# weigert/SoilMachine

Hardware: NVIDIA H100
Metric: particle-steps/sec (higher is better)
Workload: dtype f64

## Files before the change

soilmachine_b200/csrc/sm_coop.cuh:

```cuda
#pragma once
#include "sm_core.cuh"

#if defined(__CUDA_ARCH__)
#define SM_POPC(x) __popc((unsigned int)(x))
#else
#define SM_POPC(x) __builtin_popcount((unsigned int)(x))
#endif

#define SM_CW_SLOTS 18
#define SM_CW_PLUS 186u

#define SM_BUDGET_SLOTS 6

template <class B, class = void> struct CellBudgetOf { static constexpr bool value = false; };
template <class B> struct CellBudgetOf<B, decltype(void(B::kCellBudget))> { static constexpr bool value = B::kCellBudget; };

struct
#if defined(__CUDACC__)
    __align__(32)
#else
    alignas(32)
#endif
        CoopScratch {
  Sec32 win[SM_CW_SLOTS];
  double hs[2][8];
  double d;
  uint32_t u;
  unsigned char ord[2][8];
  uint32_t pad_[3];
  double acc[SM_BUDGET_SLOTS];
  double pad2_[2];
};

struct WindField {
  const float* v4;
  int nx, ny, nz;
  int dimx, dimy, scale;
};
SM_HD void wind_field_pspeed(const WindField& f, float px, float py, double height, float* ps) {
  if (!f.v4) { ps[0] = -2.0f; ps[1] = 0.0f; ps[2] = 1.0f; return; }
  const float sx = (float)f.dimx / (float)f.nx, sy = (float)f.scale / 32.0f, sz = (float)f.dimy / (float)f.nz;
  int lx = (int)(px / sx), lz = (int)(py / sz);
  int ly = (int)((float)(height * 80.0 / (double)f.scale) * (float)f.scale / sy);
  lx = lx < 0 ? 0 : (lx > f.nx - 1 ? f.nx - 1 : lx);
  ly = ly < 0 ? 0 : (ly > f.ny - 1 ? f.ny - 1 : ly);
  lz = lz < 0 ? 0 : (lz > f.nz - 1 ? f.nz - 1 : lz);
  const float* v = f.v4 + (((size_t)lx * f.ny + ly) * f.nz + lz) * 4;
  for (int k = 0; k < 3; k++) {
    float c = v[k] / 0.05f;
    c = c < -2.0f ? -2.0f : (c > 2.0f ? 2.0f : c);
    ps[k] = c;
  }
}

template <class B> struct CoopWin {
  B& b;
  CoopScratch* s;
  int ax, ay, bx, by;
  uint32_t valid, dirtym;
  bool has_b;
  float f_freq, f_track;
  static constexpr bool kBudget = B::kBudget;
  static constexpr bool kCellBudget = CellBudgetOf<B>::value;
  SM_HD CoopWin(B& b_, CoopScratch* s_) : b(b_), s(s_), ax(0), ay(0), bx(0), by(0), valid(0), dirtym(0), has_b(false),
                                          f_freq(0.f), f_track(0.f) {}
  SM_HD int dimx() const { return b.dimx(); }
  SM_HD int dimy() const { return b.dimy(); }
  SM_HD int scale() const { return b.scale(); }
  SM_HD const SoilDev& soil(uint32_t t) const { return *b.soilp(t); }

  SM_HD int slot_of(int x, int y) const {
    int dx = x - ax + 1, dy = y - ay + 1;
    if ((unsigned)dx < 3u && (unsigned)dy < 3u) return dx * 3 + dy;
    if (has_b) {
      dx = x - bx + 1; dy = y - by + 1;
      if ((unsigned)dx < 3u && (unsigned)dy < 3u) return 9 + dx * 3 + dy;
    }
    return -1;
  }
  template <class W> SM_HD void fetch_a(W& w, uint32_t want) {
    const int nx_ = b.dimx(), ny_ = b.dimy();
    const uint32_t have = valid;
    const uint32_t got = w.ballot(9, [&](int k) {
      const int x = ax + k / 3 - 1, y = ay + k % 3 - 1;
      const bool need = ((want >> k) & 1u) && !((have >> k) & 1u) && x >= 0 && y >= 0 && x < nx_ && y < ny_;
      if (need) s->win[k] = *b.cell_ptr(x, y);
      return need;
    });
    valid |= got;
  }
  template <class W> SM_HD void begin(W& w, int ix, int iy, int kind, uint32_t mask = 0x1FFu) {
    ax = ix; ay = iy; has_b = false; valid = 0; dirtym = 0;
    const int ind = iy * b.dimx() + ix;
    if (kind == 0) { f_freq = b.wfreq(ind); f_track = b.wtrack(ind); }
    else f_freq = b.windfreq(ind);
    fetch_a(w, mask);
  }
  template <class W> SM_HD void target(W& w, int nx, int ny) {
    bx = nx; by = ny; has_b = true;
    const int nx_ = b.dimx(), ny_ = b.dimy();
    const uint32_t have = valid;
    const uint32_t got = w.ballot(18, [&](int l) {
      if (l < 9) {
        const int x = nx + l / 3 - 1, y = ny + l % 3 - 1;
        bool need = x >= 0 && y >= 0 && x < nx_ && y < ny_;
        const int dx = x - ax + 1, dy = y - ay + 1;
        if ((unsigned)dx < 3u && (unsigned)dy < 3u) need = false;
        if (need) s->win[9 + l] = *b.cell_ptr(x, y);
        return need;
      }
      const int k = l - 9;
      const int x = ax + k / 3 - 1, y = ay + k % 3 - 1;
      const int dx = x - nx + 1, dy = y - ny + 1;
      const bool need = !((have >> k) & 1u) && (unsigned)dx < 3u && (unsigned)dy < 3u && x >= 0 && y >= 0 && x < nx_ && y < ny_;
      if (need) s->win[k] = *b.cell_ptr(x, y);
      return need;
    });
    valid |= ((got & 0x1FFu) << 9) | (got >> 9);
  }
  SM_HD Sec32* rec(int x, int y) {
    const int sl = slot_of(x, y);
    return sl >= 0 ? &s->win[sl] : b.cell_ptr(x, y);
  }
  SM_HD double height(int x, int y) { return rec_height(*rec(x, y)); }
  SM_HD void dirty(int x, int y) {
    const int sl = slot_of(x, y);
    if (sl >= 0) dirtym |= 1u << sl;
  }
  SM_HD void dirty_rec(const Sec32* r) {
    const long off = (long)(r - s->win);
    if (off >= 0 && off < SM_CW_SLOTS) dirtym |= 1u << (int)off;
  }
  template <class W> SM_HD void touched(W& w, Sec32* r, int x, int y) {
    dirty_rec(r);
    if (B::kHydroHooks && w.lead()) b.air_mark(r, x, y);
  }
  SM_HD void detach() { ax = ay = bx = by = -(1 << 28); has_b = false; valid = 0; dirtym = 0; }
  SM_HD void dirty_rec(Sec32* r, int x, int y) { dirty_rec(r); if (B::kHydroHooks) b.air_mark(r, x, y); }
  SM_HD void wet_mark(int x, int y) { if (B::kHydroHooks) b.wet_mark(x, y); }
  SM_HD double volume_factor() const { return b.volume_factor(); }
  SM_HD void cell_budget(int term, int x, int y, double d) {
    if constexpr (kCellBudget) b.cell_budget(term, x, y, d);
  }
  template <class W> SM_HD void flush(W& w) {
    const uint32_t m = dirtym;
    w.each(SM_CW_SLOTS, [&](int l) {
      if ((m >> l) & 1u) {
        const int ox = l < 9 ? ax : bx, oy = l < 9 ? ay : by, k = l < 9 ? l : l - 9;
        *b.cell_ptr(ox + k / 3 - 1, oy + k % 3 - 1) = s->win[l];
      }
    });
    dirtym = 0;
  }
  SM_HD void focus(int x, int y) { b.focus(x, y); }
  SM_HD Sec32 pool_load(uint32_t i) { return b.pool_load(i); }
  SM_HD void pool_store(uint32_t i, const Sec32& r) { b.pool_store(i, r); }
  SM_HD uint32_t pool_alloc() { return b.pool_alloc(); }
  SM_HD void pool_free(uint32_t i) { b.pool_free(i); }
};

template <class A>
SM_HD bool cascade_eval(A& a, const Sec32* pc, const Sec32* pn, int SCALE, float& transfer, uint32_t& cascades,
                        bool& centre_top) {
  const double dd = (rec_height(*pc) - rec_height(*pn)) * (float)SCALE;
  const Sec32* const tr = (dd > 0) ? pc : pn;
  const SoilDev& sp = a.soil(rec_surface(*tr));
  if (fabs(dd) < 80.0 * (double)sp.maxdiff * (1.0 - 9.5367431640625e-07)) return false;
  const float diff = (float)(dd / 80.0f);
  if (diff == 0) return false;
  const float excess = fabsf(diff) - sp.maxdiff;
  if (excess <= 0) return false;
  transfer = sp.settling * excess / 2.0f;
  const double tsize = (tr->type == SM_EMPTY) ? 0.0 : tr->size;
  if (transfer > tsize) transfer = (float)tsize;
  cascades = sp.cascades;
  centre_top = dd > 0;
  return true;
}

template <int DEPTH, class W, class A> struct CascadeCoop {
  static SM_HD void run(W& w, A& a, int cx, int cy, int transferloop) {
    const int dimx = a.dimx(), dimy = a.dimy();
    const int SCALE = a.scale();
    double* const hs = a.s->hs[DEPTH];
    unsigned char* const ord = a.s->ord[DEPTH];
    const unsigned int inb = ((cx > 0 ? 0x07u : 0u) | 0x18u | (cx < dimx - 1 ? 0xE0u : 0u)) &
                             ((cy > 0 ? 0x29u : 0u) | 0x42u | (cy < dimy - 1 ? 0x94u : 0u));
    const int num = SM_POPC(inb);
    Sec32* const pc = a.rec(cx, cy);
    const unsigned int active = w.ballot(8, [&](int k) {
      if (!((inb >> k) & 1u)) { hs[k] = -1.0e300; return false; }
      const int kk = k + (k >= 4 ? 1 : 0);
      const Sec32* pn = a.rec(cx + kk / 3 - 1, cy + kk % 3 - 1);
      hs[k] = rec_height(*pn);
      float t; uint32_t cs; bool ct;
      return cascade_eval(a, pc, pn, SCALE, t, cs, ct);
    });
    if (active == 0) return;
    w.each(8, [&](int k) {
      const double hk = hs[k];
      int r = 0;
#pragma unroll
      for (int j = 0; j < 8; j++) {
        const double hj = hs[j];
        r += (j > k) ? (hj > hk ? 1 : 0) : ((j < k) ? (hk > hj ? 0 : 1) : 0);
      }
      ord[r] = (unsigned char)k;
    });
    int f = -1;
#pragma unroll
    for (int r = 7; r >= 0; r--) if (r < num && ((active >> ord[r]) & 1u)) f = r;
    for (;;) {
      const int k = (int)ord[f];
      const int kk = k + (k >= 4 ? 1 : 0);
      const int nx = cx + kk / 3 - 1, ny = cy + kk % 3 - 1;
      Sec32* const pn = a.rec(nx, ny);
      w.one([&]() {
        float transfer = 0.f; uint32_t casc = 0; bool ctop = false;
        cascade_eval(a, pc, pn, SCALE, transfer, casc, ctop);
        Sec32* const tr = ctop ? pc : pn;
        Sec32* const br = ctop ? pn : pc;
        a.b.note_transfer();
        double ht0 = 0.0, hb0 = 0.0;
        if (A::kBudget) { ht0 = rec_height(*tr); hb0 = rec_height(*br); }
        a.focus(ctop ? cx : nx, ctop ? cy : ny);
        const bool re = col_remove(a, *tr, (double)transfer) != 0;
        a.focus(ctop ? nx : cx, ctop ? ny : cy);
        col_add(a, *br, (double)transfer, casc);
        if (A::kBudget) {
          const double dt = rec_height(*tr) - ht0, db = rec_height(*br) - hb0;
          a.s->acc[2] += dt + db;
          a.cell_budget(2, ctop ? cx : nx, ctop ? cy : ny, dt);
          a.cell_budget(2, ctop ? nx : cx, ctop ? ny : cy, db);
        }
        a.s->u = re ? 1u : 0u;
      });
      a.touched(w, pc, cx, cy);
      a.touched(w, pn, nx, ny);
      if constexpr (DEPTH > 0) {
        const bool recascade = a.s->u != 0;
        if (recascade && transferloop > 0) {
          --transferloop;
          CascadeCoop<DEPTH - 1, W, A>::run(w, a, nx, ny, transferloop);
        }
      }
      const int start = f + 1;
      const unsigned int act = w.ballot(num, [&](int r) {
        if (r < start) return false;
        const int k2 = (int)ord[r];
        const int kk2 = k2 + (k2 >= 4 ? 1 : 0);
        const Sec32* pn2 = a.rec(cx + kk2 / 3 - 1, cy + kk2 % 3 - 1);
        float t; uint32_t cs; bool ct;
        return cascade_eval(a, pc, pn2, SCALE, t, cs, ct);
      });
      if (act == 0) return;
      f = SM_FFS(act) - 1;
    }
  }
};

struct WaterMidCoop {
  float freq, solubility, equrate;
  double evaprate;
  int ix, iy;
};
template <class W, class A> SM_HD int water_move_coop(W& w, A& a, WaterP& p, WaterMidCoop& m, uint32_t amask = 0x1FFu) {
  const int dimx = a.dimx(), dimy = a.dimy();
  if (A::kBudget && w.lead()) { for (int k = 0; k < SM_BUDGET_SLOTS; k++) a.s->acc[k] = 0.0; }
  const int ix = (int)roundf(p.px), iy = (int)roundf(p.py);
  a.begin(w, ix, iy, 0, amask);
  const sm_f3 n = map_normal(a, ix, iy);
  Sec32* const ir = a.rec(ix, iy);
  SoilDev param = a.soil(rec_surface(*ir));
  double evaprate = 0.01;
  const int ind = iy * dimx + ix;
  if (w.lead()) a.b.set_wtrack(ind, (float)(a.f_track + p.volume));
  const float freq = a.f_freq;
  param.friction = param.friction * (1.0f - freq);
  evaprate = evaprate * (1.0f - 0.2f * freq);
  m.freq = freq; m.solubility = param.solubility; m.equrate = param.equrate; m.evaprate = evaprate;
  m.ix = ix; m.iy = iy;
  {
    const float vx = n.x * param.friction, vz = n.z * param.friction;
    if (sqrtf(vx * vx + vz * vz) < 1E-5) return SM_EXIT_STALL;
  }
  {
    const float f = param.friction;
    const float mx = n.x * (1.0f - f) + p.sx * f;
    const float my = n.z * (1.0f - f) + p.sy * f;
    const float inv = 1.0f / sqrtf(mx * mx + my * my);
    p.sx = SM_SQRT2F * (mx * inv);
    p.sy = SM_SQRT2F * (my * inv);
  }
  p.px += p.sx;
  p.py += p.sy;
  if (!(p.px >= 0.0f && p.py >= 0.0f) ||
      !(p.px < (float)dimx - 1.0f && p.py < (float)dimy - 1.0f)) {
    if (A::kBudget && w.lead()) a.s->acc[3] += p.sediment * p.volume;
    p.volume = 0.0;
    return SM_EXIT_OOB;
  }
  return SM_ALIVE;
}
template <class W, class A> SM_HD int water_interact_coop(W& w, A& a, WaterP& p, const WaterMidCoop& m) {
  const int SCALE = a.scale();
  const int ix = m.ix, iy = m.iy;
  const float freq = m.freq;
  const double evaprate = m.evaprate;
  Sec32* const ir = a.rec(ix, iy);
  const int nx = (int)roundf(p.px), ny = (int)roundf(p.py);
  a.target(w, nx, ny);
  double c_eq = m.solubility * (rec_height(*ir) - map_height_bilinear(a, p.px, p.py)) *
                (double)SCALE / 80.0;
  if (c_eq < 0.0) c_eq = 0.0;
  if (c_eq > 1.0) c_eq = 1.0;
  if ((double)(a.soil(p.contains).erosionrate) < freq)
    p.contains = a.soil(p.contains).erodes;
  const double cdiff = c_eq - p.sediment;
  if (cdiff > 0) {
    p.sediment += m.equrate * cdiff;
    p.contains = a.soil(rec_surface(*ir)).transports;
    const double amount = m.equrate * cdiff * p.volume;
    w.one([&]() {
      const double h0 = A::kBudget ? rec_height(*ir) : 0.0;
      a.focus(ix, iy);
      double diff = col_remove(a, *ir, amount);
      SM_UNROLL1
      while (fabs(diff) > 1E-8) diff = col_remove(a, *ir, diff);
      if (A::kBudget) { const double d = h0 - rec_height(*ir); a.s->acc[0] += d; a.cell_budget(0, ix, iy, d); }
    });
    a.dirty_rec(ir);
  } else if (cdiff < 0) {
    const float eq = a.soil(p.contains).equrate;
    p.sediment += eq * cdiff;
    const double amount = -eq * cdiff * p.volume;
    const uint32_t what = p.contains;
    w.one([&]() {
      const double h0 = A::kBudget ? rec_height(*ir) : 0.0;
      a.focus(ix, iy);
      col_add(a, *ir, amount, what);
      if (A::kBudget) { const double d = rec_height(*ir) - h0; a.s->acc[1] += d; a.cell_budget(1, ix, iy, d); }
    });
    a.dirty_rec(ir);
  }
  CascadeCoop<0, W, A>::run(w, a, nx, ny, 0);
// ... 2 lines not shown
  if (p.sediment > 1.0) p.sediment = 1.0;
  p.volume *= (1.0 - evaprate);
  const bool lives = p.volume > 0.01;
  if (A::kBudget && w.lead()) {
    if (over > 0.0) a.s->acc[4] += over * p.volume;
    if (!lives) a.s->acc[3] += p.sediment * p.volume;
  }
  return lives ? SM_ALIVE : SM_EXIT_EVAP;
}
template <class W, class A> SM_HD int water_step_coop(W& w, A& a, WaterP& p, uint32_t amask = 0x1FFu) {
  WaterMidCoop m;
  const int r = water_move_coop(w, a, p, m, amask);
  if (r != SM_ALIVE) return r;
  return water_interact_coop(w, a, p, m);
}

struct WindMidCoop {
  float suspension;
  uint32_t transports;
  int ix, iy;
};
template <class W, class A> SM_HD int wind_move_coop(W& w, A& a, WindP& p, WindMidCoop& m, uint32_t amask = 0x1FFu) {
  const int dimx = a.dimx(), dimy = a.dimy();
  const int SCALE = a.scale();
  if (A::kBudget && w.lead()) { for (int k = 0; k < SM_BUDGET_SLOTS; k++) a.s->acc[k] = 0.0; }
  if (a.soil(p.contains).suspension == 0.0) return SM_EXIT_OOB;
  const int ix = (int)roundf(p.px), iy = (int)roundf(p.py);
  a.begin(w, ix, iy, 1, amask);
  const sm_f3 n = map_normal(a, ix, iy);
  Sec32* const ir = a.rec(ix, iy);
  const SoilDev& param = a.soil(rec_surface(*ir));
  m.suspension = param.suspension; m.transports = param.transports; m.ix = ix; m.iy = iy;
  if (w.lead()) a.b.set_windfreq(iy * dimx + ix, (float)(0.5 * a.f_freq + 0.5f));
  const double sheight = rec_height(*ir) * (float)SCALE / 80.0f;
  if (p.height < sheight) p.height = sheight;
  if (p.height > sheight) {
    p.sy = (float)(p.sy - 0.25);
  } else {
    const sm_f3 s{p.sx, p.sy, p.sz};
    const sm_f3 v = f3_cross(f3_cross(s, n), n);
    const double wt = 0.8;
    p.sx = (float)((double)s.x * (1.0 - wt) + (double)v.x * wt);
    p.sy = (float)((double)s.y * (1.0 - wt) + (double)v.y * wt);
    p.sz = (float)((double)s.z * (1.0 - wt) + (double)v.z * wt);
  }
  {
    float ps[3];
    a.b.pspeed(p.px, p.py, p.height, ps);
    const double wt = 0.2;
    p.sx = (float)((double)p.sx * (1.0 - wt) + (double)(ps[0]) * wt);
    p.sy = (float)((double)p.sy * (1.0 - wt) + (double)(ps[1]) * wt);
    p.sz = (float)((double)p.sz * (1.0 - wt) + (double)(ps[2]) * wt);
  }
  p.px += p.sx;
  p.py += p.sz;
  p.height += p.sy;
  if (!(p.px >= 0.0f && p.py >= 0.0f) ||
      !((int)p.px < dimx - 1 && (int)p.py < dimy - 1) ||
      sqrtf(p.sx * p.sx + p.sy * p.sy + p.sz * p.sz) < 0.01) {
    if (A::kBudget && w.lead()) a.s->acc[3] += p.sediment;
    return SM_EXIT_OOB;
  }
  return SM_ALIVE;
}
template <class W, class A> SM_HD int wind_interact_coop(W& w, A& a, WindP& p, const WindMidCoop& m) {
  const int SCALE = a.scale();
  const int ix = m.ix, iy = m.iy;
// ... 64 lines not shown
```

soilmachine_b200/csrc/sm_engine.cu:

```cuda
#include <cuda_runtime.h>
#include <stddef.h>
#include <stdio.h>
#include <stdlib.h>
#include <string.h>
#include <string>
#include <vector>
#include <algorithm>
#include "../../include/soilmachine_b200.h"
#include "../../include/soilmachine/soilfile.hpp"
#include "sm_device.cuh"
#include "sm_noise.cuh"
#include "sm_hydro.cuh"
#include "sm_lbm.cuh"
#include "sm_snap.cuh"
#include "sm_layer.cuh"
#include "sm_relax.cuh"
#include <cub/device/device_scan.cuh>
#include <type_traits>

#define KIND_WATER 0
#define KIND_WIND 1

template <int KIND> struct Reach {
  static constexpr int D = (KIND == KIND_WATER) ? 6 : 10;
// ... 1163 lines not shown
  HydroAccess a(c, s_soils, s_rec, s_tag, am, true);
  HydroCount hc{};
  const unsigned long long cells = am.ncells;
  for (unsigned long long cell = active_next(am, 0); cell < cells; cell = active_next(am, cell + 1))
    hydro_seep_visit(a, (int)(cell / (unsigned long long)c.dimy), (int)(cell % (unsigned long long)c.dimy), hc);
  a.flush();
  hydro_count_out(out, hc);
}

template <bool CELLS> struct HydroCellsRef {
  __device__ __forceinline__ explicit HydroCellsRef(double*) {}
};
template <> struct HydroCellsRef<true> {
  double* hcells;
  __device__ __forceinline__ explicit HydroCellsRef(double* m) : hcells(m) {}
};
struct FreqPeers {
  float* wfreq[SM_MAX_RANKS];
  float* wtrack[SM_MAX_RANKS];
};
template <bool MULTI> struct FreqPeersRef {
  __device__ __forceinline__ explicit FreqPeersRef(const FreqPeers*) {}
};
template <> struct FreqPeersRef<true> {
  const FreqPeers* fp;
  __device__ __forceinline__ explicit FreqPeersRef(const FreqPeers* f) : fp(f) {}
};
template <bool MULTI, bool BUDGET, bool CELLS = false>
struct HydroBack : DevBack<MULTI, BUDGET>, HydroCellsRef<CELLS>, FreqPeersRef<MULTI> {
  static_assert(!CELLS || BUDGET, "the per-cell maps are measured by the budget instantiations");
  static_assert(!(CELLS && MULTI), "the hydrology's per-cell maps are not kept on a sharded map");
  static constexpr bool kHydroHooks = true;
  static constexpr bool kCellBudget = CELLS;
  ActiveMap act;
  bool marking;
  __device__ __forceinline__ HydroBack(const DevCtx& ctx, const SoilDev* ss, const ActiveMap& am, bool mk,
                                       double* cells = nullptr, const FreqPeers* fp = nullptr)
      : DevBack<MULTI, BUDGET>(ctx, ss, 0u), HydroCellsRef<CELLS>(cells), FreqPeersRef<MULTI>(fp), act(am), marking(mk) {}
  __device__ __forceinline__ float wfreq(int i) const {
    if constexpr (MULTI) return this->fp->wfreq[owner_of_x<true>(this->c, i % this->c.dimx)][i];
    else return this->c.wfreq[i];
  }
  __device__ __forceinline__ float wtrack(int i) const {
    if constexpr (MULTI) return this->fp->wtrack[owner_of_x<true>(this->c, i % this->c.dimx)][i];
    else return this->c.wtrack[i];
  }
  __device__ __forceinline__ void set_wtrack(int i, float v) {
    if constexpr (MULTI) this->fp->wtrack[owner_of_x<true>(this->c, i % this->c.dimx)][i] = v;
    else this->c.wtrack[i] = v;
  }
  __device__ __forceinline__ void cell_budget(int term, int x, int y, double d) {
    if constexpr (CELLS) {
      double* const m = this->hcells + ((size_t)x * this->c.dimy + y) * SM_HYDRO_CELL_TERMS + term;
      __builtin_assume(__isGlobal(m));
      atomicAdd(m, d);
    }
  }
  __device__ __forceinline__ void air_mark(Sec32* r, int x, int y) {
    if (marking && r->type == SM_AIR) active_mark_block(act, x, y, this->c.dimx, this->c.dimy);
  }
  __device__ __forceinline__ void wet_mark(int x, int y) {
    if (marking) active_set(act, (unsigned long long)x * this->c.dimy + y);
  }
};
struct HydroTotals {
  HydroCount hc;
// ... 835 lines not shown
  bool use_coop = SM_DEFAULT_COOP || ctx->d.bud != nullptr || ctx->d.wind_v4 != nullptr;
  {
    const char* e = getenv("SM_KERNEL");
    if (e && strcmp(e, "thread") == 0) use_coop = false;
    if (e && strcmp(e, "warp") == 0) use_coop = true;
  }
  if (ctx->d_cells && !use_coop) ctx->cells_state = 2;
  else if (ctx->d_cells && ctx->cells_state == 0) ctx->cells_state = 1;
  if (use_coop) {
    const int sw_warps = kind == KIND_WIND ? SwShape<KIND_WIND>::WARPS : SwShape<KIND_WATER>::WARPS;
    const int cthreads = sw_warps * 32;
    int occ = 0;
    const bool budget = ctx->d.bud != nullptr;
    bool exact = false;
    {
      const char* e = getenv("SM_EXACT");
      exact = (((e ? atoi(e) : SM_DEFAULT_EXACT) >> kind) & 1) != 0;
    }
    void* const fns[16] = {(void*)k_sweep<KIND_WATER, false, false, false, false>, (void*)k_sweep<KIND_WIND, false, false, false, false>,
                           (void*)k_sweep<KIND_WATER, true, false, false, false>,  (void*)k_sweep<KIND_WIND, true, false, false, false>,
                           (void*)k_sweep<KIND_WATER, false, true, false, false>,  (void*)k_sweep<KIND_WIND, false, true, false, false>,
                           (void*)k_sweep<KIND_WATER, true, true, false, false>,   (void*)k_sweep<KIND_WIND, true, true, false, false>,
                           (void*)k_sweep<KIND_WATER, false, false, true, false>,  (void*)k_sweep<KIND_WIND, false, false, true, false>,
                           (void*)k_sweep<KIND_WATER, true, false, true, false>,   (void*)k_sweep<KIND_WIND, true, false, true, false>,
                           (void*)k_sweep<KIND_WATER, false, true, true, false>,   (void*)k_sweep<KIND_WIND, false, true, true, false>,
                           (void*)k_sweep<KIND_WATER, true, true, true, false>,    (void*)k_sweep<KIND_WIND, true, true, true, false>};
    void* const fns_cells[8] = {(void*)k_sweep<KIND_WATER, false, true, false, true>, (void*)k_sweep<KIND_WIND, false, true, false, true>,
                                (void*)k_sweep<KIND_WATER, true, true, false, true>,  (void*)k_sweep<KIND_WIND, true, true, false, true>,
                                (void*)k_sweep<KIND_WATER, false, true, true, true>,  (void*)k_sweep<KIND_WIND, false, true, true, true>,
                                (void*)k_sweep<KIND_WATER, true, true, true, true>,   (void*)k_sweep<KIND_WIND, true, true, true, true>};
    void* fn = ctx->d_cells ? fns_cells[(exact ? 4 : 0) + (multi ? 2 : 0) + (kind == KIND_WATER ? 0 : 1)]
                            : fns[(exact ? 8 : 0) + (budget ? 4 : 0) + (multi ? 2 : 0) + (kind == KIND_WATER ? 0 : 1)];
    const size_t csmem = (size_t)2 * (((size_t)std::max(n, 1) + 31) / 32) * sizeof(unsigned int);
    if (csmem > 40 * 1024) CK(cudaFuncSetAttribute((const void*)fn, cudaFuncAttributeMaxDynamicSharedMemorySize, (int)csmem));
    CK(cudaOccupancyMaxActiveBlocksPerMultiprocessor(&occ, (const void*)fn, cthreads, csmem));
    if (occ < 1) return fail(ctx, SM_ERR_CUDA, "sweep kernel does not fit an SM");
    const long long maxblocks = std::max<long long>(1, (long long)ctx->num_sms * occ / ctx->share);
    const long long want = ((long long)std::max(n, 1) + sw_warps - 1) / sw_warps;
    const int cblocks = (int)std::max<long long>(1, std::min(maxblocks, want));
    DevCtx dd = ctx->d;
    int ms = max_sweeps;
    if (ms <= 0) ms = -1;
    if (max_sweeps == SM_SWEEPS_NONE) ms = 0;
    CellMaps cm = ctx->cells_of;
    void* cargs[] = {&dd, &n, (void*)&d_spawn, &ms, &cm};
    CK(cudaMemsetAsync(ctx->d.ctl, 0, 4 * sizeof(unsigned int), ctx->stream));
    CK(cudaMemsetAsync(&ctx->d.ctl->ticket[0], 0, 3 * sizeof(unsigned int), ctx->stream));
    for (int i = 0; i < 3; i++)
      CK(cudaMemsetAsync(ctx->d.lmask[i], 0, ((size_t)ctx->max_particles / 32 + 2) * sizeof(unsigned int), ctx->stream));
    CK(cudaEventRecord(ctx->ev0, ctx->stream));
    CK(cudaLaunchCooperativeKernel(fn, dim3(cblocks), dim3(cthreads), cargs, csmem, ctx->stream));
    CK(cudaEventRecord(ctx->ev1, ctx->stream));
    ctx->launches++;
    ctx->timing_pending = true;
    return SM_OK;
  }
  DevCtx d = ctx->d;
  if (max_sweeps <= 0) max_sweeps = -1;
  if (max_sweeps == SM_SWEEPS_NONE) max_sweeps = 0;
  void* args[] = {&d, &n, (void*)&d_spawn, &max_sweeps, &lshift};
  CK(cudaMemsetAsync(ctx->d.ctl, 0, 4 * sizeof(unsigned int), ctx->stream));
  CK(cudaEventRecord(ctx->ev0, ctx->stream));
  if (multi && kind == KIND_WATER)
    CK(cudaLaunchCooperativeKernel((void*)k_run<KIND_WATER, true>, dim3(blocks), dim3(threads), args, smem, ctx->stream));
  else if (multi)
    CK(cudaLaunchCooperativeKernel((void*)k_run<KIND_WIND, true>, dim3(blocks), dim3(threads), args, smem, ctx->stream));
  else if (use_exact && kind == KIND_WATER)
// ... 1200 lines not shown
```

soilmachine_b200/csrc/sm_sweep.cuh:

```cuda
#pragma once
#include "sm_coop.cuh"

template <int KIND> struct SwShape {
  static constexpr int WARPS = (KIND == KIND_WIND) ? 10 : 8;
  static constexpr int MINBLOCKS = (KIND == KIND_WIND) ? 2 : 3;
};
#define SM_SW_NEAR 31
#define SM_SW_NEARX 128

struct WarpDev {
  int lane;
  template <class F> __device__ __forceinline__ void each(int n, F f) {
    __syncwarp();
    if (lane < n) f(lane);
    __syncwarp();
  }
  template <class F> __device__ __forceinline__ unsigned int ballot(int n, F f) {
    __syncwarp();
    bool v = false;
    if (lane < n) v = f(lane);
    const unsigned int m = __ballot_sync(0xffffffffu, v);
    __syncwarp();
    return m;
  }
  template <class F> __device__ __forceinline__ void one(F f) {
    __syncwarp();
    if (lane == 0) f();
    __syncwarp();
  }
  __device__ __forceinline__ bool lead() const { return lane == 0; }
};

struct CellMaps {
  double* p[SM_MAX_RANKS];
};

template <bool CELLS> struct CellMapsRef {
  __device__ __forceinline__ explicit CellMapsRef(const CellMaps*) {}
};
template <> struct CellMapsRef<true> {
  const CellMaps* cm;
  __device__ __forceinline__ explicit CellMapsRef(const CellMaps* m) : cm(m) {}
};

template <bool MULTI, bool BUDGET = false, bool CELLS = false> struct DevBack : CellMapsRef<CELLS> {
  static constexpr bool kBudget = BUDGET;
  static constexpr bool kHydroHooks = false;
  static constexpr bool kCellBudget = CELLS;
  __device__ __forceinline__ void air_mark(Sec32*, int, int) {}
  __device__ __forceinline__ void wet_mark(int, int) {}
  __device__ __forceinline__ double volume_factor() const { return c.volume_factor; }
  const DevCtx& c;
  const SoilDev* s_soils;
  unsigned int phase;
  int cur_q;
  __device__ __forceinline__ DevBack(const DevCtx& ctx, const SoilDev* ss, unsigned int tag, const CellMaps* m = nullptr)
      : CellMapsRef<CELLS>(m), c(ctx), s_soils(ss), phase(tag % 3u), cur_q(0) {}
  __device__ __forceinline__ void cell_budget(int term, int x, int y, double d) {
    const int q = owner_of_x<MULTI>(c, x);
    double* const m = this->cm->p[q];
    atomicAdd(m + ((size_t)(x - q * c.strip_w) * c.dimy + y) * 3 + term, d);
  }
  __device__ __forceinline__ int dimx() const { return c.dimx; }
  __device__ __forceinline__ int dimy() const { return c.dimy; }
// ... 23 lines not shown
    atomicAdd(&c.ctl->drops, 1ull);
    return SM_NIL;
  }
  __device__ void pool_free(uint32_t i) {
    RunCtl* const ctl = MULTI ? c.peer[cur_q].ctl : c.ctl;
    uint32_t* const ring = MULTI ? c.peer[cur_q].ringbuf[phase] : c.ringbuf[phase];
    const unsigned long long cap = MULTI ? c.peer[cur_q].pool_cap : c.pool_cap;
    PoolRing* R = &ctl->ring[phase];
    const unsigned long long t = MULTI ? atomicAdd_system(&R->tail, 1ull) : atomicAdd(&R->tail, 1ull);
    ring[t % cap] = i;
  }
  __device__ __forceinline__ float wfreq(int i) const { return c.wfreq[i]; }
  __device__ __forceinline__ float wtrack(int i) const { return c.wtrack[i]; }
  __device__ __forceinline__ float windfreq(int i) const { return c.windfreq[i]; }
  __device__ __forceinline__ void set_wtrack(int i, float v) { c.wtrack[i] = v; }
  __device__ __forceinline__ void set_windfreq(int i, float v) { c.windfreq[i] = v; }
  __device__ __forceinline__ void note_transfer() {}
  __device__ __forceinline__ void pspeed(float px, float py, double height, float* ps) const {
    const WindField f{c.wind_v4, c.wind_nx, c.wind_ny, c.wind_nz, c.dimx, c.dimy, c.scale};
    wind_field_pspeed(f, px, py, height, ps);
  }
};

struct __align__(32) WarpSmem {
  CoopScratch cs;
  uint32_t blk[SM_SW_NEARX];
  uint32_t pred[12];
  uint32_t cnt;
  uint32_t m0[SM_SW_NEARX / 32];
  uint32_t n1[SM_SW_NEARX / 32];
  uint32_t remote;
  uint32_t succ;
  uint32_t blkxy[SM_SW_NEARX];
};

#ifndef SM_PREFETCH
#define SM_PREFETCH 1
#endif
__device__ __forceinline__ float next_dy(const WaterP& p) { return p.sy; }
__device__ __forceinline__ float next_dy(const WindP& p) { return p.sz; }
template <class W, class A> __device__ __forceinline__ int do_step_coop(W& w, A& a, WaterP& p) { return water_step_coop(w, a, p); }
template <class W, class A> __device__ __forceinline__ int do_step_coop(W& w, A& a, WindP& p) { return wind_step_coop(w, a, p); }

template <int KIND, bool MULTI, bool EXACT = false>
__device__ __forceinline__ uint32_t coop_scan(const DevCtx& c, WarpSmem& ws, int lane, unsigned int tag, int pid, int ix,
                                              int iy, int R) {
  const unsigned int par = tag & 1u;
  const int G = Reach<KIND>::G;
  const int nbx = (c.dimx + G - 1) / G, nby = (c.dimy + G - 1) / G;
  if (lane == 0) { ws.cnt = 0; ws.succ = 0; if (EXACT) ws.remote = 0; }
  if (EXACT && lane < SM_SW_NEARX / 32) ws.m0[lane] = 0;
  __syncwarp();
  if (lane < 9) {
    const int cx = ix / G + lane / 3 - 1, cy = iy / G + lane % 3 - 1;
    uint32_t best = SM_NIL;
    if (cx >= 0 && cx < nbx && cy >= 0 && cy < nby) {
      const int bq = MULTI ? owner_of_x<MULTI>(c, cx * G) : 0;
      const unsigned long long* hp = MULTI ? c.peer[bq].head[par] : c.head[par];
      const unsigned long long h = *((volatile const unsigned long long*)&hp[cx * nby + cy]);
      if ((unsigned int)(h >> 32) == tag) {
        const uint2* nodes = MULTI ? c.peer[bq].node[par] : c.node[par];
        const uint32_t qtag = MULTI ? ((uint32_t)bq << 28) : 0u;
        uint32_t j = (uint32_t)h;
        while (j != SM_NIL) {
          const uint2 nd = nodes[j];
          if (j > (uint32_t)pid) ws.succ = 1u;
// ... 241 lines not shown
  for (int i = lo; i < hi; i++) { s_pref[i] = run; run += (unsigned int)__popc(s_word[i]); }
  __syncthreads();
  return total;
}

template <int KIND, bool MULTI, bool BUDGET, bool EXACT, bool CELLS>
__global__ void __launch_bounds__(SwShape<KIND>::WARPS * 32, SwShape<KIND>::MINBLOCKS) k_sweep(DevCtx c, int n, const float* __restrict__ spawn,
                                                                            int max_sweeps, const __grid_constant__ CellMaps cm) {
  typedef typename PType<KIND>::T P;
  constexpr int NWARPS = SwShape<KIND>::WARPS;
  __shared__ SoilDev s_soils[SM_MAX_SOILS];
  __shared__ unsigned int s_alive, s_total, s_wsum[NWARPS];
  __shared__ WarpSmem s_w[NWARPS];
  extern __shared__ unsigned int s_live[];
  const int W = (n + 31) >> 5;
  unsigned int* const s_word = s_live;
  unsigned int* const s_pref = s_live + W;
  for (int i = threadIdx.x; i < c.nsoils; i += blockDim.x) s_soils[i] = c.soils[i];
  if (threadIdx.x == 0) s_alive = 0;
  __syncthreads();

  RunCtl* ctl = c.ctl;
  unsigned int epoch = 0;
  const unsigned int tag0 = ctl->tag_base;
  const unsigned int gbase = MULTI ? ctl->epoch_base : 0u;
  const int gtid = blockIdx.x * blockDim.x + threadIdx.x;
  const int lane = threadIdx.x & 31;
  const int wib = threadIdx.x >> 5;
  const int slot = blockIdx.x * NWARPS + wib;
  const int nslots = gridDim.x * NWARPS;
  WarpSmem& ws = s_w[wib];
  WarpDev w{lane};

  unsigned long long n_steps = 0, n_oob = 0, n_evap = 0, n_stall = 0;
  bool any_doa = false;

  unsigned int total_alive = 0;
  {
    unsigned int my_alive = 0;
    unsigned long long doa = 0;
    const int nthreads = gridDim.x * blockDim.x;
    for (int pid = gtid; pid < n; pid += nthreads) {
      bool alive;
      if (spawn != nullptr) {
        const float x = spawn[2 * pid], y = spawn[2 * pid + 1];
        const int sx = (int)roundf(x), sy = (int)roundf(y);
        if (MULTI && owner_of_x<MULTI>(c, sx) != c.rank) {
          c.alive[pid] = 0;
          if (BUDGET) for (int k = 0; k < SM_BUDGET_SLOTS; k++) c.bud[(size_t)pid * SM_BUDGET_SLOTS + k] = 0.0;
          continue;
        }
        const uint32_t contains = s_soils[rec_surface(*cell_ptr<MULTI>(c, sx, sy))].transports;
        if (KIND == KIND_WATER) {
          WaterP q{x, y, 0.0f, 0.0f, 1.0, 0.0, contains};
          store_particle(c, pid, q);
          alive = true;
        } else {
          WindP q{x, y, -2.0f, 0.0f, 1.0f, 0.0, 0.0, contains};
          store_particle(c, pid, q);
          alive = !(s_soils[contains].suspension == 0.0);
          if (!alive) { doa++; any_doa = true; }
        }
        c.alive[pid] = alive ? 1 : 0;
        c.done[pid] = alive ? (tag0 - 1u) : 0xFFFFFFFFu;
        if (EXACT) c.fin[pid] = alive ? (tag0 - 1u) : 0xFFFFFFFFu;
        if (BUDGET) for (int k = 0; k < SM_BUDGET_SLOTS; k++) c.bud[(size_t)pid * SM_BUDGET_SLOTS + k] = 0.0;
      } else {
// ... 17 lines not shown
    if (MULTI) total_alive = grid_barrier_x(c, epoch, gbase, 0u, true, &s_total);
    else grid_barrier(&ctl->barrier, epoch);
  }
  const bool xnb = MULTI && c.strip_w >= 3 * Reach<KIND>::G;
  bool xglobal = true;
  int last_active = -1;

  int s = 0;
  for (;; s++) {
    const unsigned int tag = tag0 + (unsigned int)s;
    if (max_sweeps >= 0 && s >= max_sweeps) {
      if (!MULTI) total_alive = live_total<NWARPS>(c.lmask[tag % 3u], W, s_word, s_pref, s_wsum);
      break;
    }
    const unsigned int live = live_total<NWARPS>(c.lmask[tag % 3u], W, s_word, s_pref, s_wsum);
    if (!MULTI) total_alive = live;
    if ((!MULTI || xglobal) && total_alive == 0) break;
    {
      unsigned int* const z = c.lmask[(tag + 2u) % 3u];
      for (int i = gtid; i < W; i += gridDim.x * blockDim.x) z[i] = 0u;
    }
    if (gtid == 0) {
      if (MULTI) st_volatile_u32(&ctl->alive_slot[(s + 2) % 3], 0u);
      st_volatile_u32(&ctl->ticket[(tag + 2u) % 3u], 0u);
    }

    unsigned int my_alive = 0;
#ifdef SM_PROFILE
    unsigned long long prof_warp = 0;
    if (gtid == 0 && s < 16380) c.dbg[8 * s + 0] = live;
#endif
    {
    for (unsigned int rank = (unsigned int)slot; rank < live;) {
      int lo = 0, hi = W - 1;
      while (lo < hi) {
        const int mid = (lo + hi + 1) >> 1;
        if (s_pref[mid] <= rank) lo = mid; else hi = mid - 1;
      }
      const int pid = (lo << 5) + (int)__fns(s_word[lo], 0u, (int)(rank - s_pref[lo]) + 1);
      last_active = s;
#ifdef SM_PROFILE
      const long long pc0 = clock64();
      if (lane == 0 && s < 16380) {
        unsigned long long gt; asm volatile("mov.u64 %0, %%globaltimer;" : "=l"(gt));
        atomicMax(&c.dbg[8 * s + 6], ~gt);
      }
#endif
      P p;
      load_particle(c, pid, p);
      const int ix = (int)roundf(p.px), iy = (int)roundf(p.py);
      const int myR = particle_reach(p);
      const uint32_t tgt = coop_scan<KIND, MULTI, EXACT>(c, ws, lane, tag, pid, ix, iy, myR);
#ifdef SM_PROFILE
      const long long pc1 = clock64();
      long long pc2 = pc1;
#endif
      bool edge = false;
      if (MULTI) {
        const int xlo = c.rank * c.strip_w, xhi = xlo + c.strip_w;
        edge = (ix < xlo + 32 && c.rank > 0) || (ix >= xhi - 32 && c.rank < c.nranks - 1);
      }
      int r = SM_ALIVE;
      bool exact_now = false;
      if constexpr (EXACT) {
        exact_now = ws.cnt <= SM_SW_NEARX && !(MULTI && ws.remote);
        if (exact_now) r = sweep_exact<KIND, MULTI, BUDGET, CELLS>(c, ws, w, s_soils, tag, pid, ix, iy, myR, p, edge, &cm);
      }
      if (!exact_now) {
        coop_wait<MULTI>(c, tag, tgt);
#ifdef SM_PROFILE
// ... 12 lines not shown
        }
#else
        r = do_step_coop(w, a, p);
#endif
        a.flush(w);
        if (lane == 0) {
          const unsigned int pub = (r == SM_ALIVE) ? tag : 0xFFFFFFFFu;
          if (ws.succ) {
            if (EXACT && !(MULTI && edge)) {
              fence_acq_rel_gpu();
              st_relaxed_u32(&c.fin[pid], pub);
              st_relaxed_u32(&c.done[pid], pub);
            } else {
              if (EXACT) st_release_u32(&c.fin[pid], pub);
              if (MULTI && edge) st_release_sys_u32(&c.done[pid], pub);
              else st_release_u32(&c.done[pid], pub);
            }
          } else {
            if (EXACT) st_volatile_u32(&c.fin[pid], pub);
            st_volatile_u32(&c.done[pid], pub);
          }
        }
#ifdef SM_PROFILE
        if (lane == 0) {
          const long long pcp = clock64();
          unsigned long long* const ph = c.dbg + 8 * 16383;
          atomicAdd(&ph[0], (unsigned long long)(pc1 - pc0));
          atomicAdd(&ph[1], (unsigned long long)(pc2 - pc1));
          atomicAdd(&ph[2], (unsigned long long)(pcm - pc2));
          atomicAdd(&ph[3], (unsigned long long)(pci - pcm));
          atomicAdd(&ph[4], (unsigned long long)(pcp - pci));
          atomicAdd(&ph[5], 1ull);
          if (ws.succ) { atomicAdd(&ph[6], (unsigned long long)(pcp - pci)); atomicAdd(&ph[7], 1ull); }
        }
#endif
      }
      const int jx = (int)roundf(p.px), jy = (int)roundf(p.py);
      if (lane == 0) {
        if (BUDGET) {
          const int bq = (MULTI && r == SM_ALIVE) ? owner_of_x<MULTI>(c, jx) : c.rank;
          double* const dst = (MULTI && bq != c.rank) ? c.peer[bq].bud : c.bud;
          for (int k = 0; k < SM_BUDGET_SLOTS; k++) {
            const size_t at = (size_t)pid * SM_BUDGET_SLOTS + k;
            const double tot = c.bud[at] + ws.cs.acc[k];
            if (MULTI && bq != c.rank) c.bud[at] = 0.0;
            dst[at] = tot;
          }
        }
        if (r == SM_ALIVE) {
          int ddx = jx - ix, ddy = jy - iy;
          ddx = ddx < 0 ? -ddx : ddx; ddy = ddy < 0 ? -ddy : ddy;
          const int lim = myR - Reach<KIND>::RING;
          if (ddx > lim || ddy > lim) atomicOr(&ctl->err, 1u << 4);
          const int nq = owner_of_x<MULTI>(c, jx);
          if (MULTI && nq != c.rank) {
            DevCtx o = c;
            o.pa = c.peer[nq].pa; o.pb = c.peer[nq].pb; o.pc = c.peer[nq].pc;
            store_particle(o, pid, p);
            c.peer[nq].done[pid] = tag;
            if (EXACT) c.peer[nq].fin[pid] = tag;
            c.peer[nq].alive[pid] = 1;
            c.alive[pid] = 0;
            atomicOr_system(&c.peer[nq].lmask[(tag + 1u) % 3u][pid >> 5], 1u << (pid & 31));
          } else {
            store_particle(c, pid, p);
            atomicOr(&c.lmask[(tag + 1u) % 3u][pid >> 5], 1u << (pid & 31));
          }
          bin_insert<KIND, MULTI>(c, tag + 1u, pid, jx, jy, particle_reach(p), nq);
        } else {
          store_particle(c, pid, p);
          c.alive[pid] = 0;
        }
      }
#if SM_PREFETCH
      if (r == SM_ALIVE && lane < 18) {
        const int ox = lane < 9 ? jx : (int)roundf(p.px + p.sx);
        const int oy = lane < 9 ? jy : (int)roundf(p.py + next_dy(p));
        const int k = lane < 9 ? lane : lane - 9;
        const int x = ox + k / 3 - 1, y = oy + k % 3 - 1;
        if (x >= 0 && y >= 0 && x < c.dimx && y < c.dimy && (!MULTI || owner_of_x<MULTI>(c, x) == c.rank))
          prefetch_l2(cell_ptr<MULTI>(c, x, y));
      }
#endif
#ifdef SM_PROFILE
      {
        const long long pc3 = clock64();
        prof_warp += (unsigned long long)(pc3 - pc0);
        if (lane == 0 && s < 16380) {
          atomicMax(&c.dbg[8 * s + 1], (unsigned long long)(pc3 - pc2));
          atomicMax(&c.dbg[8 * s + 2], (unsigned long long)(pc2 - pc1));
          atomicAdd(&c.dbg[8 * s + 4], (unsigned long long)(pc3 - pc2));
          atomicAdd(&c.dbg[8 * s + 5], 1ull);
        }
      }
#endif
      if (r == SM_ALIVE) { n_steps++; my_alive++; }
      else if (r == SM_EXIT_OOB) n_oob++;
      else if (r == SM_EXIT_STALL) n_stall++;
      else { n_steps++; n_evap++; }
      __syncwarp();
      if (live <= (unsigned int)nslots) break;
      unsigned int nr = 0;
      if (lane == 0) nr = (unsigned int)nslots + atomicAdd(&ctl->ticket[tag % 3u], 1u);
      rank = __shfl_sync(0xffffffffu, nr, 0);
    }
    }
#ifdef SM_PROFILE
    if (lane == 0 && s < 16380 && prof_warp) {
      atomicMax(&c.dbg[8 * s + 3], prof_warp);
      unsigned long long gt; asm volatile("mov.u64 %0, %%globaltimer;" : "=l"(gt));
      atomicMax(&c.dbg[8 * s + 7], gt);
    }
#endif
    if (MULTI) {
      if (lane == 0 && my_alive) atomicAdd(&s_alive, my_alive);
      __syncthreads();
      if (threadIdx.x == 0) {
        if (s_alive) atomicAdd(&ctl->alive_slot[(s + 1) % 3], s_alive);
        s_alive = 0;
      }
    }
    if (MULTI) {
      xglobal = !xnb || ((s + 1) % SM_XSYNC_K == 0) || (max_sweeps >= 0 && s + 1 >= max_sweeps);
      total_alive = grid_barrier_x(c, epoch, gbase, (unsigned int)((s + 1) % 3), xglobal, &s_total);
    } else grid_barrier(&ctl->barrier, epoch);
  }

  if (lane == 0) {
    if (n_steps) atomicAdd(&ctl->steps, n_steps);
    if (n_oob) atomicAdd(&ctl->exit_oob, n_oob);
    if (n_evap) atomicAdd(&ctl->exit_evap, n_evap);
    if (n_stall) atomicAdd(&ctl->exit_stall, n_stall);
  }
  if (any_doa) atomicMax(&ctl->sweeps, 1ull);
  if (MULTI && lane == 0 && last_active >= 0) atomicMax(&ctl->sweeps, (unsigned long long)(last_active + 1));
  if (gtid == 0) {
    if (!MULTI) atomicMax(&ctl->sweeps, (unsigned long long)s);
    ctl->alive = total_alive;
    ctl->tag_base = tag0 + (unsigned int)s + 2u;
    if (MULTI) ctl->epoch_base = gbase + epoch;
  }
}
```

Before: 196.4 million.

## Cache cell heights in window scratch and parallelize the rank search across the warp

Adds a per-slot height cache beside the staged window cells so that cascade evaluation and erosion read a precomputed height instead of walking the section stack each time. The cache is refreshed whenever a slot is marked dirty, and the hydrology backend turns it off. Cascade neighbour ordering now packs the slot index into the order byte, which avoids recomputing slot lookups. The binary search over prefix counts becomes a warp-wide radix search using ballot. Step counters move from registers into shared memory, and the dynamic shared-memory attribute check now includes static usage. The cost is extra shared memory per warp, which may lower occupancy, plus extra height recomputation on every dirty mark.

```diff
diff --git a/soilmachine_b200/csrc/sm_coop.cuh b/soilmachine_b200/csrc/sm_coop.cuh
--- a/soilmachine_b200/csrc/sm_coop.cuh
+++ b/soilmachine_b200/csrc/sm_coop.cuh
@@ -1,5 +1,8 @@
 #pragma once
 #include "sm_core.cuh"
+
+template <class W, class F> SM_HD void each_after(W& w, int n, F f) { w.each(n, f); }
+template <class W, class F> SM_HD void one_after(W& w, F f) { w.one(f); }
 
 #if defined(__CUDA_ARCH__)
 #define SM_POPC(x) __popc((unsigned int)(x))
@@ -14,6 +17,8 @@
 
 template <class B, class = void> struct CellBudgetOf { static constexpr bool value = false; };
 template <class B> struct CellBudgetOf<B, decltype(void(B::kCellBudget))> { static constexpr bool value = B::kCellBudget; };
+template <class B, class = void> struct HeightCacheOf { static constexpr bool value = true; };
+template <class B> struct HeightCacheOf<B, decltype(void(B::kHeightCache))> { static constexpr bool value = B::kHeightCache; };
 
 struct
 #if defined(__CUDACC__)
@@ -23,6 +28,7 @@
 #endif
         CoopScratch {
   Sec32 win[SM_CW_SLOTS];
+  double hwin[SM_CW_SLOTS];
   double hs[2][8];
   double d;
   uint32_t u;
@@ -62,6 +68,7 @@
   float f_freq, f_track;
   static constexpr bool kBudget = B::kBudget;
   static constexpr bool kCellBudget = CellBudgetOf<B>::value;
+  static constexpr bool kHeightCache = HeightCacheOf<B>::value;
   SM_HD CoopWin(B& b_, CoopScratch* s_) : b(b_), s(s_), ax(0), ay(0), bx(0), by(0), valid(0), dirtym(0), has_b(false),
                                           f_freq(0.f), f_track(0.f) {}
   SM_HD int dimx() const { return b.dimx(); }
@@ -78,13 +85,18 @@
     }
     return -1;
   }
+  SM_HD void stage(int sl, int x, int y) {
+    const Sec32 r = *b.cell_ptr(x, y);
+    s->win[sl] = r;
+    if constexpr (kHeightCache) s->hwin[sl] = rec_height(r);
+  }
   template <class W> SM_HD void fetch_a(W& w, uint32_t want) {
     const int nx_ = b.dimx(), ny_ = b.dimy();
     const uint32_t have = valid;
     const uint32_t got = w.ballot(9, [&](int k) {
       const int x = ax + k / 3 - 1, y = ay + k % 3 - 1;
       const bool need = ((want >> k) & 1u) && !((have >> k) & 1u) && x >= 0 && y >= 0 && x < nx_ && y < ny_;
-      if (need) s->win[k] = *b.cell_ptr(x, y);
+      if (need) stage(k, x, y);
       return need;
     });
     valid |= got;
@@ -106,30 +118,41 @@
         bool need = x >= 0 && y >= 0 && x < nx_ && y < ny_;
         const int dx = x - ax + 1, dy = y - ay + 1;
         if ((unsigned)dx < 3u && (unsigned)dy < 3u) need = false;
-        if (need) s->win[9 + l] = *b.cell_ptr(x, y);
+        if (need) stage(9 + l, x, y);
         return need;
       }
       const int k = l - 9;
       const int x = ax + k / 3 - 1, y = ay + k % 3 - 1;
       const int dx = x - nx + 1, dy = y - ny + 1;
       const bool need = !((have >> k) & 1u) && (unsigned)dx < 3u && (unsigned)dy < 3u && x >= 0 && y >= 0 && x < nx_ && y < ny_;
-      if (need) s->win[k] = *b.cell_ptr(x, y);
+      if (need) stage(k, x, y);
       return need;
     });
     valid |= ((got & 0x1FFu) << 9) | (got >> 9);
   }
-  SM_HD Sec32* rec(int x, int y) {
+  SM_HD Sec32* rec_at(int sl, int x, int y) { return sl >= 0 ? &s->win[sl] : b.cell_ptr(x, y); }
+  SM_HD Sec32* rec(int x, int y) { return rec_at(slot_of(x, y), x, y); }
+  SM_HD double height_at(int sl, const Sec32* r) const {
+    if constexpr (kHeightCache) return sl >= 0 ? s->hwin[sl] : rec_height(*r);
+    return rec_height(*r);
+  }
+  SM_HD double height(int x, int y) {
     const int sl = slot_of(x, y);
-    return sl >= 0 ? &s->win[sl] : b.cell_ptr(x, y);
-  }
-  SM_HD double height(int x, int y) { return rec_height(*rec(x, y)); }
+    return height_at(sl, rec_at(sl, x, y));
+  }
   SM_HD void dirty(int x, int y) {
     const int sl = slot_of(x, y);
-    if (sl >= 0) dirtym |= 1u << sl;
+    if (sl >= 0) {
+      dirtym |= 1u << sl;
+      if constexpr (kHeightCache) s->hwin[sl] = rec_height(s->win[sl]);
+    }
   }
   SM_HD void dirty_rec(const Sec32* r) {
     const long off = (long)(r - s->win);
-    if (off >= 0 && off < SM_CW_SLOTS) dirtym |= 1u << (int)off;
+    if (off >= 0 && off < SM_CW_SLOTS) {
+      dirtym |= 1u << (int)off;
+      if constexpr (kHeightCache) s->hwin[off] = rec_height(*r);
+    }
   }
   template <class W> SM_HD void touched(W& w, Sec32* r, int x, int y) {
     dirty_rec(r);
@@ -160,9 +183,9 @@
 };
 
 template <class A>
-SM_HD bool cascade_eval(A& a, const Sec32* pc, const Sec32* pn, int SCALE, float& transfer, uint32_t& cascades,
-                        bool& centre_top) {
-  const double dd = (rec_height(*pc) - rec_height(*pn)) * (float)SCALE;
+SM_HD bool cascade_eval(A& a, const Sec32* pc, const Sec32* pn, double hc, double hn, int SCALE, float& transfer,
+                        uint32_t& cascades, bool& centre_top) {
+  const double dd = (hc - hn) * (float)SCALE;
   const Sec32* const tr = (dd > 0) ? pc : pn;
   const SoilDev& sp = a.soil(rec_surface(*tr));
   if (fabs(dd) < 80.0 * (double)sp.maxdiff * (1.0 - 9.5367431640625e-07)) return false;
@@ -187,17 +210,21 @@
     const unsigned int inb = ((cx > 0 ? 0x07u : 0u) | 0x18u | (cx < dimx - 1 ? 0xE0u : 0u)) &
                              ((cy > 0 ? 0x29u : 0u) | 0x42u | (cy < dimy - 1 ? 0x94u : 0u));
     const int num = SM_POPC(inb);
-    Sec32* const pc = a.rec(cx, cy);
+    const int csl = a.slot_of(cx, cy);
+    Sec32* const pc = a.rec_at(csl, cx, cy);
     const unsigned int active = w.ballot(8, [&](int k) {
       if (!((inb >> k) & 1u)) { hs[k] = -1.0e300; return false; }
       const int kk = k + (k >= 4 ? 1 : 0);
-      const Sec32* pn = a.rec(cx + kk / 3 - 1, cy + kk % 3 - 1);
-      hs[k] = rec_height(*pn);
+      const int nx = cx + kk / 3 - 1, ny = cy + kk % 3 - 1;
+      const int sl = a.slot_of(nx, ny);
+      const Sec32* pn = a.rec_at(sl, nx, ny);
+      const double hn = a.height_at(sl, pn);
+      hs[k] = hn;
       float t; uint32_t cs; bool ct;
-      return cascade_eval(a, pc, pn, SCALE, t, cs, ct);
+      return cascade_eval(a, pc, pn, a.height_at(csl, pc), hn, SCALE, t, cs, ct);
     });
     if (active == 0) return;
-    w.each(8, [&](int k) {
+    each_after(w, 8, [&](int k) {
       const double hk = hs[k];
       int r = 0;
 #pragma unroll
@@ -205,19 +232,20 @@
         const double hj = hs[j];
         r += (j > k) ? (hj > hk ? 1 : 0) : ((j < k) ? (hk > hj ? 0 : 1) : 0);
       }
-      ord[r] = (unsigned char)k;
+      const int kk = k + (k >= 4 ? 1 : 0);
+      ord[r] = (unsigned char)(k | ((a.slot_of(cx + kk / 3 - 1, cy + kk % 3 - 1) + 1) << 3));
     });
     int f = -1;
 #pragma unroll
-    for (int r = 7; r >= 0; r--) if (r < num && ((active >> ord[r]) & 1u)) f = r;
+    for (int r = 7; r >= 0; r--) if (r < num && ((active >> (ord[r] & 7u)) & 1u)) f = r;
     for (;;) {
-      const int k = (int)ord[f];
+      const int k = (int)(ord[f] & 7u), sl = (int)(ord[f] >> 3) - 1;
       const int kk = k + (k >= 4 ? 1 : 0);
       const int nx = cx + kk / 3 - 1, ny = cy + kk % 3 - 1;
-      Sec32* const pn = a.rec(nx, ny);
-      w.one([&]() {
+      Sec32* const pn = a.rec_at(sl, nx, ny);
+      one_after(w, [&]() {
         float transfer = 0.f; uint32_t casc = 0; bool ctop = false;
-        cascade_eval(a, pc, pn, SCALE, transfer, casc, ctop);
+        cascade_eval(a, pc, pn, a.height_at(csl, pc), a.height_at(sl, pn), SCALE, transfer, casc, ctop);
         Sec32* const tr = ctop ? pc : pn;
         Sec32* const br = ctop ? pn : pc;
         a.b.note_transfer();
@@ -247,11 +275,11 @@
       const int start = f + 1;
       const unsigned int act = w.ballot(num, [&](int r) {
         if (r < start) return false;
-        const int k2 = (int)ord[r];
+        const int k2 = (int)(ord[r] & 7u), sl2 = (int)(ord[r] >> 3) - 1;
         const int kk2 = k2 + (k2 >= 4 ? 1 : 0);
-        const Sec32* pn2 = a.rec(cx + kk2 / 3 - 1, cy + kk2 % 3 - 1);
+        const Sec32* pn2 = a.rec_at(sl2, cx + kk2 / 3 - 1, cy + kk2 % 3 - 1);
         float t; uint32_t cs; bool ct;
-        return cascade_eval(a, pc, pn2, SCALE, t, cs, ct);
+        return cascade_eval(a, pc, pn2, a.height_at(csl, pc), a.height_at(sl2, pn2), SCALE, t, cs, ct);
       });
       if (act == 0) return;
       f = SM_FFS(act) - 1;
@@ -310,7 +338,7 @@
   Sec32* const ir = a.rec(ix, iy);
   const int nx = (int)roundf(p.px), ny = (int)roundf(p.py);
   a.target(w, nx, ny);
-  double c_eq = m.solubility * (rec_height(*ir) - map_height_bilinear(a, p.px, p.py)) *
+  double c_eq = m.solubility * (a.height(ix, iy) - map_height_bilinear(a, p.px, p.py)) *
                 (double)SCALE / 80.0;
   if (c_eq < 0.0) c_eq = 0.0;
   if (c_eq > 1.0) c_eq = 1.0;
@@ -379,7 +407,7 @@
   const SoilDev& param = a.soil(rec_surface(*ir));
   m.suspension = param.suspension; m.transports = param.transports; m.ix = ix; m.iy = iy;
   if (w.lead()) a.b.set_windfreq(iy * dimx + ix, (float)(0.5 * a.f_freq + 0.5f));
-  const double sheight = rec_height(*ir) * (float)SCALE / 80.0f;
+  const double sheight = a.height(ix, iy) * (float)SCALE / 80.0f;
   if (p.height < sheight) p.height = sheight;
   if (p.height > sheight) {
     p.sy = (float)(p.sy - 0.25);
diff --git a/soilmachine_b200/csrc/sm_engine.cu b/soilmachine_b200/csrc/sm_engine.cu
--- a/soilmachine_b200/csrc/sm_engine.cu
+++ b/soilmachine_b200/csrc/sm_engine.cu
@@ -1219,6 +1219,7 @@
   static_assert(!(CELLS && MULTI), "the hydrology's per-cell maps are not kept on a sharded map");
   static constexpr bool kHydroHooks = true;
   static constexpr bool kCellBudget = CELLS;
+  static constexpr bool kHeightCache = false;
   ActiveMap act;
   bool marking;
   __device__ __forceinline__ HydroBack(const DevCtx& ctx, const SoilDev* ss, const ActiveMap& am, bool mk,
@@ -2120,7 +2121,10 @@
     void* fn = ctx->d_cells ? fns_cells[(exact ? 4 : 0) + (multi ? 2 : 0) + (kind == KIND_WATER ? 0 : 1)]
                             : fns[(exact ? 8 : 0) + (budget ? 4 : 0) + (multi ? 2 : 0) + (kind == KIND_WATER ? 0 : 1)];
     const size_t csmem = (size_t)2 * (((size_t)std::max(n, 1) + 31) / 32) * sizeof(unsigned int);
-    if (csmem > 40 * 1024) CK(cudaFuncSetAttribute((const void*)fn, cudaFuncAttributeMaxDynamicSharedMemorySize, (int)csmem));
+    cudaFuncAttributes fa;
+    CK(cudaFuncGetAttributes(&fa, (const void*)fn));
+    if (fa.sharedSizeBytes + csmem > 48 * 1024)
+      CK(cudaFuncSetAttribute((const void*)fn, cudaFuncAttributeMaxDynamicSharedMemorySize, (int)csmem));
     CK(cudaOccupancyMaxActiveBlocksPerMultiprocessor(&occ, (const void*)fn, cthreads, csmem));
     if (occ < 1) return fail(ctx, SM_ERR_CUDA, "sweep kernel does not fit an SM");
     const long long maxblocks = std::max<long long>(1, (long long)ctx->num_sms * occ / ctx->share);
diff --git a/soilmachine_b200/csrc/sm_sweep.cuh b/soilmachine_b200/csrc/sm_sweep.cuh
--- a/soilmachine_b200/csrc/sm_sweep.cuh
+++ b/soilmachine_b200/csrc/sm_sweep.cuh
@@ -30,6 +30,14 @@
   }
   __device__ __forceinline__ bool lead() const { return lane == 0; }
 };
+template <class F> __device__ __forceinline__ void each_after(WarpDev& w, int n, F f) {
+  if (w.lane < n) f(w.lane);
+  __syncwarp();
+}
+template <class F> __device__ __forceinline__ void one_after(WarpDev& w, F f) {
+  if (w.lane == 0) f();
+  __syncwarp();
+}
 
 struct CellMaps {
   double* p[SM_MAX_RANKS];
@@ -119,6 +127,7 @@
   uint32_t remote;
   uint32_t succ;
   uint32_t blkxy[SM_SW_NEARX];
+  unsigned long long nst[4];
 };
 
 #ifndef SM_PREFETCH
@@ -426,7 +435,7 @@
   WarpSmem& ws = s_w[wib];
   WarpDev w{lane};
 
-  unsigned long long n_steps = 0, n_oob = 0, n_evap = 0, n_stall = 0;
+  if (lane == 0) for (int k = 0; k < 4; k++) ws.nst[k] = 0;
   bool any_doa = false;
 
   unsigned int total_alive = 0;
@@ -510,10 +519,14 @@
 #endif
     {
     for (unsigned int rank = (unsigned int)slot; rank < live;) {
-      int lo = 0, hi = W - 1;
-      while (lo < hi) {
-        const int mid = (lo + hi + 1) >> 1;
-        if (s_pref[mid] <= rank) lo = mid; else hi = mid - 1;
+      int lo = 0;
+      for (int span = W;;) {
+        const int step = (span + 31) >> 5;
+        const bool le = lane * step < span && s_pref[lo + lane * step] <= rank;
+        const int top = 31 - __clz((int)__ballot_sync(0xffffffffu, le));
+        lo += top * step;
+        if (step == 1) break;
+        span = min(step, span - top * step);
       }
       const int pid = (lo << 5) + (int)__fns(s_word[lo], 0u, (int)(rank - s_pref[lo]) + 1);
       last_active = s;
@@ -592,6 +605,13 @@
           atomicAdd(&ph[4], (unsigned long long)(pcp - pci));
           atomicAdd(&ph[5], 1ull);
           if (ws.succ) { atomicAdd(&ph[6], (unsigned long long)(pcp - pci)); atomicAdd(&ph[7], 1ull); }
+          unsigned long long* const pb = c.dbg + 8 * (live > 2u * (unsigned int)nslots ? 16380 : (8u * live <= (unsigned int)nslots ? 16382 : 16381));
+          atomicAdd(&pb[0], (unsigned long long)(pc1 - pc0));
+          atomicAdd(&pb[1], (unsigned long long)(pc2 - pc1));
+          atomicAdd(&pb[2], (unsigned long long)(pcm - pc2));
+          atomicAdd(&pb[3], (unsigned long long)(pci - pcm));
+          atomicAdd(&pb[4], (unsigned long long)(pcp - pci));
+          atomicAdd(&pb[5], 1ull);
         }
 #endif
       }
@@ -654,10 +674,13 @@
         }
       }
 #endif
-      if (r == SM_ALIVE) { n_steps++; my_alive++; }
-      else if (r == SM_EXIT_OOB) n_oob++;
-      else if (r == SM_EXIT_STALL) n_stall++;
-      else { n_steps++; n_evap++; }
+      if (r == SM_ALIVE) my_alive++;
+      if (lane == 0) {
+        if (r == SM_ALIVE) ws.nst[0]++;
+        else if (r == SM_EXIT_OOB) ws.nst[1]++;
+        else if (r == SM_EXIT_STALL) ws.nst[3]++;
+        else { ws.nst[0]++; ws.nst[2]++; }
+      }
       __syncwarp();
       if (live <= (unsigned int)nslots) break;
       unsigned int nr = 0;
@@ -687,10 +710,10 @@
   }
 
   if (lane == 0) {
-    if (n_steps) atomicAdd(&ctl->steps, n_steps);
-    if (n_oob) atomicAdd(&ctl->exit_oob, n_oob);
-    if (n_evap) atomicAdd(&ctl->exit_evap, n_evap);
-    if (n_stall) atomicAdd(&ctl->exit_stall, n_stall);
+    if (ws.nst[0]) atomicAdd(&ctl->steps, ws.nst[0]);
+    if (ws.nst[1]) atomicAdd(&ctl->exit_oob, ws.nst[1]);
+    if (ws.nst[2]) atomicAdd(&ctl->exit_evap, ws.nst[2]);
+    if (ws.nst[3]) atomicAdd(&ctl->exit_stall, ws.nst[3]);
   }
   if (any_doa) atomicMax(&ctl->sweeps, 1ull);
   if (MULTI && lane == 0 && last_active >= 0) atomicMax(&ctl->sweeps, (unsigned long long)(last_active + 1));
```

New measurement: 212.3 million (median of 6 runs). 1.08x the previous value.
